# TengdaHan/CoCLR

Measured on AMD Instinct MI355X. Metric: clips/sec (whole node) S3D-InfoNCE seq_len=32 bs=32/GPU, higher is better.
Workload: dtype fp32

## Files before the change

coclr_amd/csrc/pool.hip:

```cpp
#include "common.h"
#include "../../include/coclr_hip.h"
#include <math.h>
#include <cstdlib>

namespace {

struct PoolGeom {
  int N, C;
  int Ti, Hi, Wi, To, Ho, Wo;
  int kt, kh, kw, st, sh, sw, pt, ph, pw;
  long x_nstride, y_nstride;
  const float* in_scale;
  const float* in_shift;
  int in_relu;
  int C0;
  int tfold;
  int nt;
};

typedef float pool_f32x4 __attribute__((ext_vector_type(4)));

__device__ __forceinline__ float4 pool_ld4(const float* p, int i, bool nt) {
  if (nt) {
    const pool_f32x4 t = __builtin_nontemporal_load(reinterpret_cast<const pool_f32x4*>(p) + i);
    return make_float4(t.x, t.y, t.z, t.w);
  }
  return reinterpret_cast<const float4*>(p)[i];
}
__device__ __forceinline__ void pool_st4(float* p, int i, const float4& w, bool nt) {
  if (nt) {
    pool_f32x4 t; t.x = w.x; t.y = w.y; t.z = w.z; t.w = w.w;
    __builtin_nontemporal_store(t, reinterpret_cast<pool_f32x4*>(p) + i);
  } else {
    reinterpret_cast<float4*>(p)[i] = w;
  }
}
inline long pool_nt_bytes() {
  const char* e = getenv("COCLR_BN_NT_MB");
  const long mb = e ? atol(e) : 0;
  return mb < 0 ? -1 : (mb << 20);
}

__device__ __forceinline__ float pool_in(const PoolGeom& g, float v, int c) {
  if (g.in_scale) {
    v = fmaf(v, g.in_scale[c], g.in_shift[c]);
    if (g.in_relu) v = fmaxf(v, 0.f);
  }
  return v;
}

__global__ void __launch_bounds__(256)
maxpool3d_fwd_kernel(const float* __restrict__ x, float* __restrict__ y, int* __restrict__ idx,
                     const PoolGeom g) {
  const int So = g.To * g.Ho * g.Wo, Si = g.Ti * g.Hi * g.Wi;
  const int planes = g.N * g.C;
  for (int pl = blockIdx.y; pl < planes; pl += gridDim.y) {
    const int n = pl / g.C, c = pl - n * g.C;
    const float* xp = x + (long)n * g.x_nstride + (long)c * Si;
    float* yp = y + (long)n * g.y_nstride + (long)c * So;
    int* ip = idx ? idx + (long)pl * So : nullptr;
    for (int o = blockIdx.x * 256 + threadIdx.x; o < So; o += gridDim.x * 256) {
      const int ow = o % g.Wo;
      const int q = o / g.Wo;
      const int oh = q % g.Ho, ot = q / g.Ho;
      int t0 = ot * g.st - g.pt, h0 = oh * g.sh - g.ph, w0 = ow * g.sw - g.pw;
      const int t1 = min(t0 + g.kt, g.Ti), h1 = min(h0 + g.kh, g.Hi), w1 = min(w0 + g.kw, g.Wi);
      t0 = max(t0, 0); h0 = max(h0, 0); w0 = max(w0, 0);
      float best = -INFINITY;
      int bi = (t0 * g.Hi + h0) * g.Wi + w0;
      for (int t = t0; t < t1; ++t)
        for (int h = h0; h < h1; ++h)
          for (int w = w0; w < w1; ++w) {
            const int ii = (t * g.Hi + h) * g.Wi + w;
            const float v = pool_in(g, xp[ii], c);
            if (v > best || v != v) { best = v; bi = ii; }
          }
      yp[o] = best;
      if (ip) ip[o] = bi;
    }
  }
}

__device__ __forceinline__ int first_out(int a, int s) { return a < 0 ? 0 : a / s + 1; }

__global__ void __launch_bounds__(256)
maxpool3d_bwd_kernel(const float* __restrict__ dy, const int* __restrict__ idx, float* dx,
                     const PoolGeom g, long dy_nstride, long dx_nstride, int accumulate) {
  const int So = g.To * g.Ho * g.Wo, Si = g.Ti * g.Hi * g.Wi;
  const int planes = g.N * g.C;
  for (int pl = blockIdx.y; pl < planes; pl += gridDim.y) {
    const int n = pl / g.C, c = pl - n * g.C;
    const float* dyp = dy + (long)n * dy_nstride + (long)c * So;
    const int* ip = idx + (long)pl * So;
    float* dxp = dx + (long)n * dx_nstride + (long)c * Si;
    for (int i = blockIdx.x * 256 + threadIdx.x; i < Si; i += gridDim.x * 256) {
      const int iw = i % g.Wi;
      const int q = i / g.Wi;
      const int ih = q % g.Hi, it = q / g.Hi;
      const int ot0 = first_out(it + g.pt - g.kt, g.st);
      const int oh0 = first_out(ih + g.ph - g.kh, g.sh);
      const int ow0 = first_out(iw + g.pw - g.kw, g.sw);
      const int ot1 = min(g.To - 1, (it + g.pt) / g.st);
      const int oh1 = min(g.Ho - 1, (ih + g.ph) / g.sh);
      const int ow1 = min(g.Wo - 1, (iw + g.pw) / g.sw);
      float s = 0.f;
      for (int ot = ot0; ot <= ot1; ++ot)
        for (int oh = oh0; oh <= oh1; ++oh)
          for (int ow = ow0; ow <= ow1; ++ow) {
            const int o = (ot * g.Ho + oh) * g.Wo + ow;
            if (ip[o] == i) s += dyp[o];
          }
      dxp[i] = accumulate ? dxp[i] + s : s;
    }
  }
}

template <int KT, int KH, int KW, int ST, int SH, int SW, int WPT, bool WITH_IDX>
__global__ void __launch_bounds__(256)
maxpool3d_tiled_fwd_kernel(const float* __restrict__ x, float* __restrict__ y,
                           int* __restrict__ idx, const PoolGeom g, int G, int planes, int tfold,
                           int vec) {
  extern __shared__ float tile[];
  const int Si = g.Ti * g.Hi * g.Wi, So = g.To * g.Ho * g.Wo;
  const int pl0 = blockIdx.x * G;
  const int gcount = min(G, planes - pl0);
  for (int gi = 0; gi < gcount; ++gi) {
    const int pl = pl0 + gi;
    const int n = pl / g.C, c = pl - n * g.C;
    const float* xp = x + (long)n * g.x_nstride + (long)c * Si;
    float* tp = tile + gi * Si;
    const int ch = c / g.tfold;
    if (vec) {
      for (int i = threadIdx.x; i < (Si >> 2); i += 256) {
        float4 v = pool_ld4(xp, i, g.nt != 0);
        v.x = pool_in(g, v.x, ch); v.y = pool_in(g, v.y, ch);
        v.z = pool_in(g, v.z, ch); v.w = pool_in(g, v.w, ch);
        reinterpret_cast<float4*>(tp)[i] = v;
      }
    } else {
      for (int i = threadIdx.x; i < Si; i += 256) tp[i] = pool_in(g, xp[i], ch);
    }
  }
  __syncthreads();
  constexpr int NR = (WPT - 1) * SW + KW;
  const int OWC = (g.Wo + WPT - 1) / WPT;
  const int rows = g.To * g.Ho;
  const int items = gcount * rows * OWC;
  for (int it = threadIdx.x; it < items; it += 256) {
    const int owc = it % OWC;
    int r = it / OWC;
    const int oh = r % g.Ho; r /= g.Ho;
    const int ot = r % g.To;
    const int gi = r / g.To;
    const int ow0 = owc * WPT;
    const float* tp = tile + gi * Si;
    float best[WPT];
    int bi[WPT];
    const int t0 = ot * ST - g.pt, h0 = oh * SH - g.ph, w0 = ow0 * SW - g.pw;
#pragma unroll
    for (int j = 0; j < WPT; ++j) {
      best[j] = -INFINITY;
      const int tt = max(t0, 0), hh = max(h0, 0), ww = max(w0 + j * SW, 0);
      bi[j] = (tt * g.Hi + hh) * g.Wi + ww;
    }
#pragma unroll
    for (int kt = 0; kt < KT; ++kt) {
      const int t = t0 + kt;
      if (t < 0 || t >= g.Ti) continue;
#pragma unroll
      for (int kh = 0; kh < KH; ++kh) {
        const int h = h0 + kh;
        if (h < 0 || h >= g.Hi) continue;
        const int rowoff = (t * g.Hi + h) * g.Wi;
        float v[NR];
#pragma unroll
        for (int q = 0; q < NR; ++q) {
          const int w = w0 + q;
          v[q] = (w >= 0 && w < g.Wi) ? tp[rowoff + w] : -INFINITY;
        }
#pragma unroll
        for (int j = 0; j < WPT; ++j) {
#pragma unroll
          for (int kw = 0; kw < KW; ++kw) {
            const float val = v[j * SW + kw];
            if (val > best[j] || val != val) { best[j] = val; bi[j] = rowoff + w0 + j * SW + kw; }
          }
        }
      }
    }
    const int pl = pl0 + gi;
    const int n = pl / g.C, c = pl - n * g.C;
    const long obase = ((long)ot * g.Ho + oh) * g.Wo + ow0;
    float* yp = y + (long)n * g.y_nstride + (long)c * So + obase;
#pragma unroll
    for (int j = 0; j < WPT; ++j) {
      if (ow0 + j < g.Wo) {
        yp[j] = best[j];
        if (WITH_IDX) idx[(long)pl * So + obase + j] = bi[j] + (pl % tfold) * Si;
      }
    }
  }
}

template <int PT, int PH, int PW, int KQ>
struct ClassLoads {
  int i[PT * PH * PW][KQ];
  int b[PT * PH * PW][KQ];
  float v[PT * PH * PW][KQ];
};

template <int PT, int PH, int PW, int KQ>
__device__ __forceinline__ void class_load(ClassLoads<PT, PH, PW, KQ>& L, const float* __restrict__ dy,
                                           const int* __restrict__ idx, const PoolGeom& g,
                                           long dy_nstride, int pl0, int gcount, int tfold, int Si,
                                           int So) {
#pragma unroll
  for (int ct = 0; ct < PT; ++ct)
#pragma unroll
    for (int ch = 0; ch < PH; ++ch)
#pragma unroll
      for (int cw = 0; cw < PW; ++cw) {
        const int cls = (ct * PH + ch) * PW + cw;
        const int nt = (g.To - ct + PT - 1) / PT, nh = (g.Ho - ch + PH - 1) / PH,
                  nw = (g.Wo - cw + PW - 1) / PW;
        const int csize = (nt > 0 && nh > 0 && nw > 0) ? nt * nh * nw : 0;
#pragma unroll
        for (int k = 0; k < KQ; ++k) {
          const int q = threadIdx.x + k * 256;
          L.i[cls][k] = -1;
          L.b[cls][k] = 0;
          L.v[cls][k] = 0.f;
          if (q < gcount * csize) {
            const int gi = q / csize;
            int m = q - gi * csize;
            const int a = m / (nh * nw);
            m -= a * nh * nw;
            const int b = m / nw, cc = m - b * nw;
            const int o = ((a * PT + ct) * g.Ho + (b * PH + ch)) * g.Wo + (cc * PW + cw);
            const int pl = pl0 + gi;
            const int n = pl / g.C, c = pl - n * g.C;
            L.b[cls][k] = gi * Si - (pl % tfold) * Si;
            L.i[cls][k] = idx[(long)pl * So + o];
            L.v[cls][k] = dy[(long)n * dy_nstride + (long)c * So + o];
          }
        }
      }
}

template <int PT, int PH, int PW, int KQ>
__device__ __forceinline__ void class_apply(const ClassLoads<PT, PH, PW, KQ>& L, float* tile) {
#pragma unroll
  for (int cls = 0; cls < PT * PH * PW; ++cls) {
    asm volatile("s_waitcnt lgkmcnt(0)\n\ts_barrier" ::: "memory");
#pragma unroll
    for (int k = 0; k < KQ; ++k)
      if (L.i[cls][k] >= 0) tile[L.b[cls][k] + L.i[cls][k]] += L.v[cls][k];
  }
}

__device__ __forceinline__ void class_scatter_generic(float* tile, const float* __restrict__ dy,
                                                      const int* __restrict__ idx, const PoolGeom& g,
                                                      long dy_nstride, int pl0, int gcount, int tfold,
                                                      int Si, int So) {
  const int Pt = (g.kt + g.st - 1) / g.st, Ph = (g.kh + g.sh - 1) / g.sh, Pw = (g.kw + g.sw - 1) / g.sw;
  for (int ct = 0; ct < Pt; ++ct)
    for (int ch = 0; ch < Ph; ++ch)
      for (int cw = 0; cw < Pw; ++cw) {
        __syncthreads();
        const int nt = (g.To - ct + Pt - 1) / Pt, nh = (g.Ho - ch + Ph - 1) / Ph,
                  nw = (g.Wo - cw + Pw - 1) / Pw;
        if (nt <= 0 || nh <= 0 || nw <= 0) continue;
        const int csize = nt * nh * nw;
        for (int q = threadIdx.x; q < gcount * csize; q += 256) {
          const int gi = q / csize;
          int m = q - gi * csize;
          const int a = m / (nh * nw);
          m -= a * nh * nw;
          const int b = m / nw, cc = m - b * nw;
          const int o = ((a * Pt + ct) * g.Ho + (b * Ph + ch)) * g.Wo + (cc * Pw + cw);
          const int pl = pl0 + gi;
          const int n = pl / g.C, c = pl - n * g.C;
          const int i = idx[(long)pl * So + o] - (pl % tfold) * Si;
          tile[gi * Si + i] += dy[(long)n * dy_nstride + (long)c * So + o];
        }
      }
}

template <int PT, int PH, int PW, int KQ>
__global__ void __launch_bounds__(256)
maxpool3d_tiled_bwd_kernel(const float* __restrict__ dy, const int* __restrict__ idx, float* dx,
                           const PoolGeom g, long dy_nstride, long dx_nstride, int accumulate,
                           int G, int planes, int tfold, int vec) {
  extern __shared__ float tile[];
  const int Si = g.Ti * g.Hi * g.Wi, So = g.To * g.Ho * g.Wo;
  const int pl0 = blockIdx.x * G;
  const int gcount = min(G, planes - pl0);
  if constexpr (PT > 0) {
    ClassLoads<PT, PH, PW, KQ> L;
    class_load<PT, PH, PW, KQ>(L, dy, idx, g, dy_nstride, pl0, gcount, tfold, Si, So);
    for (int i = threadIdx.x; i < gcount * Si; i += 256) tile[i] = 0.f;
    class_apply<PT, PH, PW, KQ>(L, tile);
  } else {
    for (int i = threadIdx.x; i < gcount * Si; i += 256) tile[i] = 0.f;
    class_scatter_generic(tile, dy, idx, g, dy_nstride, pl0, gcount, tfold, Si, So);
  }
  __syncthreads();
  for (int gi = 0; gi < gcount; ++gi) {
    const int pl = pl0 + gi;
    const int n = pl / g.C, c = pl - n * g.C;
    float* dxp = dx + (long)n * dx_nstride + (long)c * Si;
    const float* tp = tile + gi * Si;
    if (vec) {
      for (int i = threadIdx.x; i < (Si >> 2); i += 256) {
        float4 v = reinterpret_cast<const float4*>(tp)[i];
        if (accumulate) {
          const float4 o = reinterpret_cast<const float4*>(dxp)[i];
          v.x += o.x; v.y += o.y; v.z += o.z; v.w += o.w;
        }
        reinterpret_cast<float4*>(dxp)[i] = v;
      }
    } else {
      for (int i = threadIdx.x; i < Si; i += 256) dxp[i] = accumulate ? dxp[i] + tp[i] : tp[i];
    }
  }
}


struct PoolBest { float v; int i; };

__device__ __forceinline__ void pool_take(PoolBest& b, float cv, int ci) {
  if (cv > b.v || cv != cv) { b.v = cv; b.i = ci; }
}

template <bool WITH_IDX, int TT>
__global__ void __launch_bounds__(256)
maxpool333_kernel(const float* __restrict__ x, float* __restrict__ y, int* __restrict__ idx,
                  const PoolGeom g, int planes, int lW, int lHW, int vec) {
  extern __shared__ float lds[];
  const int T = TT > 0 ? TT : g.Ti;
  const int W = 1 << lW, HW = 1 << lHW, H = HW >> lW;
  const int PG = 256 >> lHW, S = T << lHW;
  float* xs = lds;
  float* bv = xs + PG * S;
  int* bi = reinterpret_cast<int*>(bv + PG * S);
  const int tid = threadIdx.x;
  const int pl0 = blockIdx.x * PG;
  const int gcount = min(PG, planes - pl0);
  if (vec) {
    const int S4 = S >> 2, total4 = gcount * S4;
    for (int e0 = tid; e0 < total4; e0 += 4 * 256) {
      float4 r[4];
      int chn[4];
#pragma unroll
      for (int k = 0; k < 4; ++k) {
        const int e = e0 + k * 256;
        chn[k] = -1;
        if (e < total4) {
          const int gi = e / S4, i = e - gi * S4;
          const int pl = pl0 + gi;
          const int n = pl / g.C, c = pl - n * g.C;
          r[k] = reinterpret_cast<const float4*>(x + (long)n * g.x_nstride + (long)c * S)[i];
          chn[k] = c;
        }
      }
#pragma unroll
      for (int k = 0; k < 4; ++k) {
        if (chn[k] < 0) continue;
        float4 v = r[k];
        v.x = pool_in(g, v.x, chn[k]); v.y = pool_in(g, v.y, chn[k]);
        v.z = pool_in(g, v.z, chn[k]); v.w = pool_in(g, v.w, chn[k]);
        reinterpret_cast<float4*>(xs)[e0 + k * 256] = v;
      }
    }
  } else {
    for (int gi = 0; gi < gcount; ++gi) {
      const int pl = pl0 + gi;
      const int n = pl / g.C, c = pl - n * g.C;
      const float* xp = x + (long)n * g.x_nstride + (long)c * S;
      float* tp = xs + gi * S;
      for (int i = tid; i < S; i += 256) tp[i] = pool_in(g, xp[i], c);
    }
  }
  __syncthreads();
  const int gl = tid >> lHW, p = tid & (HW - 1), h = p >> lW, w = p & (W - 1);
  const bool live = gl < gcount;
  if (live) {
#pragma unroll
    for (int t = 0; t < T; ++t) {
      const int row = (gl * T + t) * HW + h * W;
      const int frow = (t * H + h) * W;
      PoolBest b;
      b.v = -INFINITY;
      b.i = frow + (w > 0 ? w - 1 : 0);
      if (w > 0) pool_take(b, xs[row + w - 1], frow + w - 1);
      pool_take(b, xs[row + w], frow + w);
      if (w < W - 1) pool_take(b, xs[row + w + 1], frow + w + 1);
      bv[row + w] = b.v;
      if (WITH_IDX) bi[row + w] = b.i;
    }
  }
  __syncthreads();
  if (!live) return;
  auto plane_best = [&](int t) {
    const int col = (gl * T + t) * HW + w;
    const int h0 = h > 0 ? h - 1 : 0;
    PoolBest b;
    b.v = -INFINITY;
    b.i = WITH_IDX ? bi[col + h0 * W] : 0;
    if (h > 0) pool_take(b, bv[col + (h - 1) * W], WITH_IDX ? bi[col + (h - 1) * W] : 0);
    pool_take(b, bv[col + h * W], WITH_IDX ? bi[col + h * W] : 0);
    if (h < H - 1) pool_take(b, bv[col + (h + 1) * W], WITH_IDX ? bi[col + (h + 1) * W] : 0);
    return b;
  };
  const int pl = pl0 + gl;
  const int n = pl / g.C, c = pl - n * g.C;
  float* yp = y + (long)n * g.y_nstride + (long)c * S;
  int* ip = WITH_IDX ? idx + (long)pl * S : nullptr;
  PoolBest prev, cur = plane_best(0), next = cur;
  prev.v = -INFINITY; prev.i = cur.i;
#pragma unroll
  for (int t = 0; t < T; ++t) {
    if (t + 1 < T) next = plane_best(t + 1);
    PoolBest b;
    b.v = -INFINITY;
    b.i = t > 0 ? prev.i : cur.i;
    if (t > 0) pool_take(b, prev.v, prev.i);
    pool_take(b, cur.v, cur.i);
    if (t + 1 < T) pool_take(b, next.v, next.i);
    yp[t * HW + p] = b.v;
    if (WITH_IDX) ip[t * HW + p] = b.i;
    prev = cur;
    cur = next;
  }
}

__global__ void __launch_bounds__(256)
bn_pool_bwd_reduce_kernel(const float* __restrict__ pdy, const int* __restrict__ pidx,
                          const float* __restrict__ y, const float* __restrict__ scale,
                          const float* __restrict__ shift, const float* __restrict__ mean,
                          const float* __restrict__ invstd, double* sums, int C, int So, int Si,
                          long pdy_nstride, long y_nstride, int relu) {
  __shared__ double red[4];
  const int c = blockIdx.x, n = blockIdx.y;
  const float sc = scale[c], sf = shift[c], mu = mean[c], is = invstd[c];
  const float* dp = pdy + (long)n * pdy_nstride + (long)c * So;
  const int* ip = pidx + ((long)n * C + c) * So;
  const float* yp = y + (long)n * y_nstride + (long)c * Si;
  float ag = 0.f, agx = 0.f;
  for (int o0 = threadIdx.x; o0 < So; o0 += 1024) {
    int ii[4];
    float gg[4], vv[4];
#pragma unroll
    for (int k = 0; k < 4; ++k) {
      const int o = o0 + k * 256;
      ii[k] = o < So ? ip[o] : 0;
      gg[k] = o < So ? dp[o] : 0.f;
    }
#pragma unroll
    for (int k = 0; k < 4; ++k) vv[k] = yp[ii[k]];
#pragma unroll
    for (int k = 0; k < 4; ++k) {
      if (o0 + k * 256 >= So) break;
      float g = gg[k];
      const float v = vv[k];
      if (relu) g = fmaf(v, sc, sf) > 0.f ? g : 0.f;
      ag += g;
      agx += g * ((v - mu) * is);
    }
  }
  double sg = block256_sum_d((double)ag, red);
  double sgx = block256_sum_d((double)agx, red);
  if (threadIdx.x == 0) {
    sums[((long)c * gridDim.y + n) * 2] = sg;
    sums[((long)c * gridDim.y + n) * 2 + 1] = sgx;
  }
}

template <int PT, int PH, int PW, int KQ>
__global__ void __launch_bounds__(256)
bn_pool_bwd_apply_kernel(const float* __restrict__ pdy, const int* __restrict__ pidx,
                         const float* __restrict__ y, const float* __restrict__ scale,
                         const float* __restrict__ shift, const float* __restrict__ mean,
                         const float* __restrict__ invstd, const double* __restrict__ sums, int groups,
                         double count, int training, float* dgamma, float* dbeta, float* dy,
                         const PoolGeom g, long pdy_nstride, long y_nstride, long dy_nstride, int relu,
                         int G, int planes, int tfold, int vec) {
  extern __shared__ float tile[];
  __shared__ double tot[2];
  __shared__ float coef[8][4];
  const int Si = g.Ti * g.Hi * g.Wi, So = g.To * g.Ho * g.Wo;
  const int pl0 = blockIdx.x * G;
  const int gcount = min(G, planes - pl0);
  ClassLoads<(PT > 0 ? PT : 1), (PT > 0 ? PH : 1), (PT > 0 ? PW : 1), (PT > 0 ? KQ : 1)> L;
  if constexpr (PT > 0)
    class_load<PT, PH, PW, KQ>(L, pdy, pidx, g, pdy_nstride, pl0, gcount, tfold, Si, So);
  for (int i = threadIdx.x; i < gcount * Si; i += 256) tile[i] = 0.f;
  int cprev = -1;
  for (int gi = 0; gi < gcount; ++gi) {
    const int pl = pl0 + gi;
    const int c = (pl % g.C) / tfold;
    if (c == cprev && !(pl / g.C == 0 && (pl % g.C) % tfold == 0)) {
      if (threadIdx.x == 0)
        for (int j = 0; j < 3; ++j) coef[gi][j] = coef[gi - 1][j];
      continue;
    }
    cprev = c;
    __syncthreads();
    if (threadIdx.x < 64) {
      double a0 = 0.0, a1 = 0.0;
      for (int k = threadIdx.x; k < groups; k += 64) {
        a0 += sums[((long)c * groups + k) * 2];
        a1 += sums[((long)c * groups + k) * 2 + 1];
      }
      a0 = wave_sum_d(a0);
      a1 = wave_sum_d(a1);
      if (threadIdx.x == 0) { tot[0] = a0; tot[1] = a1; }
    }
    __syncthreads();
    if (threadIdx.x == 0) {
      const double sg = tot[0], sgx = tot[1];
      const float sc = scale[c];
      float A = sc, B = 0.f, D = 0.f;
      if (training) {
        const float mg = (float)(sg / count), mgx = (float)(sgx / count);
        B = -sc * invstd[c] * mgx;
        D = sc * (mean[c] * invstd[c] * mgx - mg);
      }
      coef[gi][0] = A; coef[gi][1] = B; coef[gi][2] = D;
      if (pl / g.C == 0 && (pl % g.C) % tfold == 0) {
        if (dgamma) dgamma[c] = (float)sgx;
        if (dbeta) dbeta[c] = (float)sg;
      }
    }
  }
  if constexpr (PT > 0) class_apply<PT, PH, PW, KQ>(L, tile);
  else class_scatter_generic(tile, pdy, pidx, g, pdy_nstride, pl0, gcount, tfold, Si, So);
  __syncthreads();
  for (int gi = 0; gi < gcount; ++gi) {
    const int pl = pl0 + gi;
    const int n = pl / g.C, c = pl - n * g.C;
    const int ch = c / tfold;
    const float A = coef[gi][0], B = coef[gi][1], D = coef[gi][2];
    const float sc = scale[ch], sf = shift[ch];
    const float* yp = y + (long)n * y_nstride + (long)c * Si;
    float* dyp = dy + (long)n * dy_nstride + (long)c * Si;
    const float* tp = tile + gi * Si;
    if (vec) {
      for (int i = threadIdx.x; i < (Si >> 2); i += 256) {
        float4 gq = reinterpret_cast<const float4*>(tp)[i];
        const float4 v = pool_ld4(yp, i, g.nt != 0);
        if (relu) {
          gq.x = fmaf(v.x, sc, sf) > 0.f ? gq.x : 0.f; gq.y = fmaf(v.y, sc, sf) > 0.f ? gq.y : 0.f;
          gq.z = fmaf(v.z, sc, sf) > 0.f ? gq.z : 0.f; gq.w = fmaf(v.w, sc, sf) > 0.f ? gq.w : 0.f;
        }
        float4 o;
        o.x = fmaf(A, gq.x, fmaf(B, v.x, D)); o.y = fmaf(A, gq.y, fmaf(B, v.y, D));
        o.z = fmaf(A, gq.z, fmaf(B, v.z, D)); o.w = fmaf(A, gq.w, fmaf(B, v.w, D));
        pool_st4(dyp, i, o, g.nt != 0);
      }
    } else {
      for (int i = threadIdx.x; i < Si; i += 256) {
        float gv = tp[i];
        const float v = yp[i];
        if (relu) gv = fmaf(v, sc, sf) > 0.f ? gv : 0.f;
        dyp[i] = fmaf(A, gv, fmaf(B, v, D));
      }
    }
  }
}

__global__ void __launch_bounds__(256)
maxpool333_bwd_kernel(const float* __restrict__ dy, const int* __restrict__ idx, float* dx,
                      const PoolGeom g, long dy_nstride, long dx_nstride, int accumulate, int G,
                      int planes, int lW, int lHW, int vec) {
  extern __shared__ float lds[];
  const int T = g.Ti, W = 1 << lW, HW = 1 << lHW, H = HW >> lW;
  const int S = T << lHW;
  float* dys = lds;
  int* ids = reinterpret_cast<int*>(lds + G * S);
  const int pl0 = blockIdx.x * G;
  const int gcount = min(G, planes - pl0);
  for (int gi = 0; gi < gcount; ++gi) {
    const int pl = pl0 + gi;
    const int n = pl / g.C, c = pl - n * g.C;
    const float* dyp = dy + (long)n * dy_nstride + (long)c * S;
    const int* ip = idx + (long)pl * S;
    if (vec) {
      for (int i = threadIdx.x; i < (S >> 2); i += 256) {
        reinterpret_cast<float4*>(dys + gi * S)[i] = reinterpret_cast<const float4*>(dyp)[i];
        reinterpret_cast<int4*>(ids + gi * S)[i] = reinterpret_cast<const int4*>(ip)[i];
      }
    } else {
      for (int i = threadIdx.x; i < S; i += 256) { dys[gi * S + i] = dyp[i]; ids[gi * S + i] = ip[i]; }
    }
  }
  __syncthreads();
  for (int q = threadIdx.x; q < gcount * S; q += 256) {
    const int gi = q / S, i = q - gi * S;
    const int t = i >> lHW, h = (i >> lW) & (H - 1), w = i & (W - 1);
    const float* dv = dys + gi * S;
    const int* iv = ids + gi * S;
    float s = 0.f;
#pragma unroll
    for (int dt = -1; dt <= 1; ++dt) {
      if (t + dt < 0 || t + dt >= T) continue;
#pragma unroll
      for (int dh = -1; dh <= 1; ++dh) {
        if (h + dh < 0 || h + dh >= H) continue;
#pragma unroll
        for (int dw = -1; dw <= 1; ++dw) {
          if (w + dw < 0 || w + dw >= W) continue;
          const int o = i + dt * HW + dh * W + dw;
          if (iv[o] == i) s += dv[o];
        }
      }
    }
    const int pl = pl0 + gi;
    const int n = pl / g.C, c = pl - n * g.C;
    float* d = dx + (long)n * dx_nstride + (long)c * S + i;
    *d = accumulate ? *d + s : s;
  }
}

constexpr int kTileFloats = 16384;

inline int pick_group(int planes, int Si) {
  if (Si > kTileFloats) return 0;
  int G = 4096 / Si;
  if (G < 1) G = 1;
  while (G > 1 && (planes + G - 1) / G < 2048) G >>= 1;
  return G;
}

template <int KT, int KH, int KW, int ST, int SH, int SW, int WPT>
int launch_tiled_fwd(const PoolGeom& g, const float* x, float* y, int* idx, int G, int planes,
                     int tfold, int vec, hipStream_t stream) {
  const size_t lds = (size_t)G * g.Ti * g.Hi * g.Wi * sizeof(float);
  const int blocks = (planes + G - 1) / G;
  if (idx) {
    auto k = maxpool3d_tiled_fwd_kernel<KT, KH, KW, ST, SH, SW, WPT, true>;
    static std::atomic<uint64_t> done{0};
    COCLR_RETURN_IF(ensure_dyn_lds(reinterpret_cast<const void*>(k), kTileFloats * 4, done));
    hipLaunchKernelGGL(k, dim3(blocks), dim3(256), lds, stream, x, y, idx, g, G, planes, tfold, vec);
  } else {
    auto k = maxpool3d_tiled_fwd_kernel<KT, KH, KW, ST, SH, SW, WPT, false>;
    static std::atomic<uint64_t> done{0};
    COCLR_RETURN_IF(ensure_dyn_lds(reinterpret_cast<const void*>(k), kTileFloats * 4, done));
    hipLaunchKernelGGL(k, dim3(blocks), dim3(256), lds, stream, x, y, idx, g, G, planes, tfold, vec);
  }
  COCLR_LAUNCH_CHECK();
  return 0;
}

inline PoolGeom fold_time(PoolGeom g) {
  if (g.kt == 1 && g.st == 1 && g.pt == 0 && g.Ti == g.To) {
    g.C = g.C * g.Ti;
    g.tfold = g.Ti;
    g.Ti = g.To = 1;
  }
  return g;
}

__global__ void __launch_bounds__(256)
global_avgpool_fwd_kernel(const float* __restrict__ x, float* __restrict__ y, int planes, int S) {
  const int wave = (blockIdx.x * 256 + threadIdx.x) >> 6, lane = threadIdx.x & 63;
  if (wave >= planes) return;
  const float* xp = x + (long)wave * S;
  float s = 0.f;
  for (int i = lane; i < S; i += 64) s += xp[i];
  s = wave_sum(s);
  if (lane == 0) y[wave] = s / (float)S;
}

__global__ void __launch_bounds__(256)
global_avgpool_bwd_kernel(const float* __restrict__ dy, float* __restrict__ dx, long total, int S) {
  const float inv = 1.f / (float)S;
  for (long e = (long)blockIdx.x * 256 + threadIdx.x; e < total; e += (long)gridDim.x * 256)
    dx[e] = dy[e / S] * inv;
}

inline dim3 pool_grid(int planes, int elems) {
  int gx = cdiv(elems, 256 * 2);
  if (gx < 1) gx = 1;
  if (gx > 128) gx = 128;
  int gy = planes > 65535 ? 65535 : planes;
  while ((long)gx * gy > 262144 && gx > 1) gx >>= 1;
  return dim3(gx, gy);
}

inline PoolGeom to_geom(const coclr_pool_desc* d) {
  PoolGeom g;
  g.N = d->N; g.C = d->C;
  g.Ti = d->Ti; g.Hi = d->Hi; g.Wi = d->Wi; g.To = d->To; g.Ho = d->Ho; g.Wo = d->Wo;
  g.kt = d->kt; g.kh = d->kh; g.kw = d->kw; g.st = d->st; g.sh = d->sh; g.sw = d->sw;
  g.pt = d->pt; g.ph = d->ph; g.pw = d->pw;
  g.x_nstride = d->x_nstride; g.y_nstride = d->y_nstride;
  g.in_scale = g.in_shift = nullptr; g.in_relu = 0; g.C0 = d->C; g.tfold = 1;
  {
    static const long nt_bytes = pool_nt_bytes();
    g.nt = (nt_bytes >= 0 && (long)d->N * d->C * d->Ti * d->Hi * d->Wi * 4 >= nt_bytes) ? 1 : 0;
  }
  return g;
}

}

static inline int ilog2_exact(int v) {
  int l = 0;
  while ((1 << l) < v) ++l;
  return (1 << l) == v ? l : -1;
}

namespace {

enum { kFwdGeneric = 0, kFwdSep333 = 1, kFwdTiled = 2 };
enum { kBwdGeneric = 0, kBwdGather333 = 1, kBwdClasses = 2 };

inline bool is_333_s1_p1(const PoolGeom& g) {
  return g.kt == 3 && g.kh == 3 && g.kw == 3 && g.st == 1 && g.sh == 1 && g.sw == 1 && g.pt == 1 && g.ph == 1 &&
         g.pw == 1;
}

struct PoolFwdPlan {
  int family;
  int tmpl;
  int G;
  int gx, gy;
  int tfold;
  int vec;
  int lds;
  int lW, lHW;
  int planes;
  PoolGeom g;
};

inline PoolFwdPlan plan_pool_fwd(const PoolGeom& g, bool with_idx) {
  PoolFwdPlan p;
  p.family = kFwdGeneric; p.tmpl = 0; p.G = 1; p.tfold = 1; p.vec = 0; p.lds = 0; p.lW = p.lHW = 0;
  p.planes = g.N * g.C;
  p.g = g;
  if (is_333_s1_p1(g)) {
    const int lW = ilog2_exact(g.Wi), lHW = ilog2_exact(g.Hi * g.Wi);
    if (lW >= 0 && lHW >= 4 && lHW <= 8 && g.Ti <= 32) {
      const int PG = 256 >> lHW, S = g.Ti << lHW;
      const size_t lds = (size_t)PG * S * 4 * (with_idx ? 3 : 2);
      if (lds <= 64 * 1024) {
        p.family = kFwdSep333;
        p.tmpl = (g.Ti == 16 || g.Ti == 8 || g.Ti == 4) ? g.Ti : 0;
        p.G = PG; p.gx = cdiv(p.planes, PG); p.gy = 1;
        p.vec = (g.x_nstride & 3) == 0;
        p.lds = (int)lds; p.lW = lW; p.lHW = lHW;
        return p;
      }
    }
  }
  {
    const PoolGeom f = fold_time(g);
    const int Si = f.Ti * f.Hi * f.Wi;
    const int planes = f.N * f.C;
    const int G = pick_group(planes, Si);
    if (G > 0) {
      const int k[3] = {f.kt, f.kh, f.kw}, s[3] = {f.st, f.sh, f.sw};
#define POOL_IS(a, b, c, e, ff, gg) (k[0] == a && k[1] == b && k[2] == c && s[0] == e && s[1] == ff && s[2] == gg)
      int row = -1;
      if (POOL_IS(1, 3, 3, 1, 2, 2)) row = 0;
      else if (POOL_IS(3, 3, 3, 1, 1, 1)) row = 1;
      else if (POOL_IS(3, 3, 3, 2, 2, 2)) row = 2;
      else if (POOL_IS(2, 2, 2, 2, 2, 2)) row = 3;
#undef POOL_IS
      if (row >= 0) {
        p.family = kFwdTiled; p.tmpl = row; p.G = G; p.gx = (planes + G - 1) / G; p.gy = 1;
        p.tfold = f.Ti == g.Ti ? 1 : g.Ti;
        p.vec = (Si & 3) == 0 && (f.x_nstride & 3) == 0;
        p.lds = (int)((size_t)G * Si * sizeof(float));
        p.planes = planes;
        p.g = f;
        return p;
      }
    }
  }
  const dim3 grid = pool_grid(g.N * g.C, g.To * g.Ho * g.Wo);
  p.gx = (int)grid.x; p.gy = (int)grid.y;
  return p;
}

}

extern "C" int coclr_maxpool3d_fwd(const coclr_pool_desc* d, const float* x, float* y,
                                   int32_t* indices, const float* in_scale, const float* in_shift,
                                   int in_relu, void* stream) {
  if (!d || d->N <= 0 || d->C <= 0) return COCLR_EINVAL;
  if (d->pt * 2 > d->kt || d->ph * 2 > d->kh || d->pw * 2 > d->kw) return COCLR_EINVAL;
  if ((in_scale == nullptr) != (in_shift == nullptr)) return COCLR_EINVAL;
  PoolGeom g = to_geom(d);
  g.in_scale = in_scale; g.in_shift = in_shift; g.in_relu = in_relu;
  const PoolFwdPlan p = plan_pool_fwd(g, indices != nullptr);
  hipStream_t st = (hipStream_t)stream;
  if (p.family == kFwdSep333) {
    const dim3 grid(p.gx);
    const size_t lds = (size_t)p.lds;
    const int planes = p.planes, lW = p.lW, lHW = p.lHW;
#define POOL333(TT)                                                                                  \
    if (indices) hipLaunchKernelGGL((maxpool333_kernel<true, TT>), grid, dim3(256), lds, st, x, y, \
                                    indices, g, planes, lW, lHW, p.vec);                         \
    else hipLaunchKernelGGL((maxpool333_kernel<false, TT>), grid, dim3(256), lds, st, x, y,       \
                            indices, g, planes, lW, lHW, p.vec)
    if (p.tmpl == 16) { POOL333(16); }
    else if (p.tmpl == 8) { POOL333(8); }
    else if (p.tmpl == 4) { POOL333(4); }
    else { POOL333(0); }
#undef POOL333
    COCLR_LAUNCH_CHECK();
    return 0;
  }
  if (p.family == kFwdTiled) {
    switch (p.tmpl) {
      case 0: return launch_tiled_fwd<1, 3, 3, 1, 2, 2, 2>(p.g, x, y, indices, p.G, p.planes, p.tfold, p.vec, st);
      case 1: return launch_tiled_fwd<3, 3, 3, 1, 1, 1, 4>(p.g, x, y, indices, p.G, p.planes, p.tfold, p.vec, st);
      case 2: return launch_tiled_fwd<3, 3, 3, 2, 2, 2, 2>(p.g, x, y, indices, p.G, p.planes, p.tfold, p.vec, st);
      default: return launch_tiled_fwd<2, 2, 2, 2, 2, 2, 2>(p.g, x, y, indices, p.G, p.planes, p.tfold, p.vec, st);
    }
  }
  hipLaunchKernelGGL(maxpool3d_fwd_kernel, dim3(p.gx, p.gy), dim3(256), 0, st, x, y, indices, g);
  COCLR_LAUNCH_CHECK();
  return 0;
}

struct ClassShape { int pt, ph, pw, kq; };
inline ClassShape class_shape(const PoolGeom& g, int G) {
  ClassShape c;
  c.pt = (g.kt + g.st - 1) / g.st; c.ph = (g.kh + g.sh - 1) / g.sh; c.pw = (g.kw + g.sw - 1) / g.sw;
  const long m = (long)((g.To + c.pt - 1) / c.pt) * ((g.Ho + c.ph - 1) / c.ph) * ((g.Wo + c.pw - 1) / c.pw);
  c.kq = (int)((G * m + 255) / 256);
  static const bool off = getenv("COCLR_POOL_PRELOAD") && atoi(getenv("COCLR_POOL_PRELOAD")) == 0;
  if (off) c.kq = 1 << 20;
  return c;
}

template <int PT, int PH, int PW, int KQ>
int launch_tiled_bwd(const float* dy, const int32_t* indices, float* dx, const PoolGeom& g,
                     long dy_nstride, long dx_nstride, int accumulate, int G, int planes, int tfold,
                     int Si, int vec, hipStream_t st) {
  auto kern = maxpool3d_tiled_bwd_kernel<PT, PH, PW, KQ>;
  static std::atomic<uint64_t> done{0};
  COCLR_RETURN_IF(ensure_dyn_lds(reinterpret_cast<const void*>(kern), kTileFloats * 4, done));
  hipLaunchKernelGGL(kern, dim3((planes + G - 1) / G), dim3(256), (size_t)G * Si * sizeof(float), st,
                     dy, indices, dx, g, dy_nstride, dx_nstride, accumulate, G, planes, tfold, vec);
  COCLR_LAUNCH_CHECK();
  return 0;
}

namespace {

struct ClassTemplate { int pt, ph, pw, kq; };
constexpr ClassTemplate kBwdTemplates[4] = {{1, 2, 2, 1}, {3, 3, 3, 1}, {2, 2, 2, 1}, {1, 1, 1, 2}};
constexpr ClassTemplate kPooledTemplates[2] = {{1, 2, 2, 1}, {2, 2, 2, 1}};

inline int pick_class_template(const ClassShape& cs, const ClassTemplate* rows, int n) {
  for (int i = 0; i < n; ++i)
    if (cs.pt == rows[i].pt && cs.ph == rows[i].ph && cs.pw == rows[i].pw && cs.kq <= rows[i].kq) return i;
  return -1;
}

struct PoolBwdPlan {
  int family;
  int tmpl;
  int G, kq;
  int gx, gy;
  int tfold;
  int vec;
  int lds;
  int lW, lHW;
  int planes, Si;
  PoolGeom g;
};

inline PoolBwdPlan plan_pool_bwd(const PoolGeom& g0, long dy_nstride, long dx_nstride) {
  PoolBwdPlan p;
  p.family = kBwdGeneric; p.tmpl = -1; p.G = 1; p.kq = 0; p.tfold = 1; p.vec = 0; p.lds = 0; p.lW = p.lHW = 0;
  p.planes = g0.N * g0.C; p.Si = g0.Ti * g0.Hi * g0.Wi;
  p.g = g0;
  if (is_333_s1_p1(g0)) {
    const int lW = ilog2_exact(g0.Wi), lHW = ilog2_exact(g0.Hi * g0.Wi);
    const int S = g0.Ti * g0.Hi * g0.Wi;
    if (lW >= 0 && lHW >= 0 && S <= 128) {
      const int planes = g0.N * g0.C;
      int G = 2048 / S;
      if (G < 1) G = 1;
      while (G > 1 && (planes + G - 1) / G < 2048) G >>= 1;
      p.family = kBwdGather333; p.G = G; p.gx = (planes + G - 1) / G; p.gy = 1;
      p.vec = (S & 3) == 0 && (dy_nstride & 3) == 0;
      p.lds = G * S * 8; p.lW = lW; p.lHW = lHW;
      return p;
    }
  }
  {
    const PoolGeom g = fold_time(g0);
    const int Si = g.Ti * g.Hi * g.Wi;
    const int planes = g.N * g.C;
    if (pick_group(planes, Si) > 0) {
      int G = 4096 / Si > 0 ? 4096 / Si : 1;
      while (G > 1 && (planes + G - 1) / G < 1024) G >>= 1;
      const ClassShape cs = class_shape(g, G);
      p.family = kBwdClasses; p.tmpl = pick_class_template(cs, kBwdTemplates, 4);
      p.G = G; p.kq = cs.kq; p.gx = (planes + G - 1) / G; p.gy = 1;
      p.tfold = g.Ti == g0.Ti ? 1 : g0.Ti;
      p.vec = (Si & 3) == 0 && (dx_nstride & 3) == 0;
      p.lds = (int)((size_t)G * Si * sizeof(float));
      p.planes = planes; p.Si = Si;
      p.g = g;
      return p;
    }
  }
  const dim3 grid = pool_grid(g0.N * g0.C, g0.Ti * g0.Hi * g0.Wi);
  p.gx = (int)grid.x; p.gy = (int)grid.y;
  return p;
}

struct PooledBnPlan {
  int fits;
  int tmpl;
  int G, kq, blocks, tfold, vec, lds, planes, Si;
  PoolGeom g;
};

inline PooledBnPlan plan_pooled_bn(const PoolGeom& g0, long y_nstride, long dy_nstride) {
  PooledBnPlan p;
  const PoolGeom g = fold_time(g0);
  p.g = g;
  p.tfold = g.Ti == g0.Ti ? 1 : g0.Ti;
  p.Si = g.Ti * g.Hi * g.Wi;
  p.planes = g.N * g.C;
  p.fits = p.Si <= kTileFloats;
  p.tmpl = -1; p.G = 0; p.kq = 0; p.blocks = 0; p.vec = 0; p.lds = 0;
  if (!p.fits) return p;
  int G = 4096 / p.Si > 0 ? 4096 / p.Si : 1;
  if (G > 8) G = 8;
  while (G > 1 && (p.planes + G - 1) / G < 1024) G >>= 1;
  const ClassShape cs = class_shape(g, G);
  p.tmpl = pick_class_template(cs, kPooledTemplates, 2);
  p.G = G; p.kq = cs.kq; p.blocks = (p.planes + G - 1) / G;
  p.vec = (p.Si & 3) == 0 && ((y_nstride | dy_nstride) & 3) == 0;
  p.lds = (int)((size_t)G * p.Si * sizeof(float));
  return p;
}

}

extern "C" int coclr_maxpool3d_bwd(const coclr_pool_desc* d, const float* dy, const int32_t* indices,
                                   float* dx, int64_t dy_nstride, int64_t dx_nstride,
                                   int accumulate, void* stream) {
  if (!d || d->N <= 0 || d->C <= 0) return COCLR_EINVAL;
  const PoolGeom g0 = to_geom(d);
  const PoolBwdPlan p = plan_pool_bwd(g0, (long)dy_nstride, (long)dx_nstride);
  hipStream_t st = (hipStream_t)stream;
  if (p.family == kBwdGather333) {
    hipLaunchKernelGGL(maxpool333_bwd_kernel, dim3(p.gx), dim3(256), (size_t)p.lds, st, dy, indices, dx, g0,
                       (long)dy_nstride, (long)dx_nstride, accumulate, p.G, p.planes, p.lW, p.lHW, p.vec);
    COCLR_LAUNCH_CHECK();
    return 0;
  }
  if (p.family == kBwdClasses) {
#define POOL_BWD(a, b, c, q)                                                                         \
    return launch_tiled_bwd<a, b, c, q>(dy, indices, dx, p.g, (long)dy_nstride, (long)dx_nstride,    \
                                        accumulate, p.G, p.planes, p.tfold, p.Si, p.vec, st)
    switch (p.tmpl) {
      case 0: POOL_BWD(1, 2, 2, 1);
      case 1: POOL_BWD(3, 3, 3, 1);
      case 2: POOL_BWD(2, 2, 2, 1);
      case 3: POOL_BWD(1, 1, 1, 2);
      default: POOL_BWD(0, 0, 0, 0);
    }
#undef POOL_BWD
  }
  hipLaunchKernelGGL(maxpool3d_bwd_kernel, dim3(p.gx, p.gy), dim3(256), 0, st, dy, indices, dx, g0,
                     (long)dy_nstride, (long)dx_nstride, accumulate);
  COCLR_LAUNCH_CHECK();
  return 0;
}

extern "C" int coclr_bn_act_backward_pooled_fits(const coclr_pool_desc* d, int* fits) {
  if (!d || !fits || d->N <= 0 || d->C <= 0) return COCLR_EINVAL;
  *fits = plan_pooled_bn(to_geom(d), 0, 0).fits;
  return 0;
}

extern "C" int coclr_bn_act_backward_pooled(const coclr_pool_desc* d, const float* pool_dy,
                                            const int32_t* pool_idx, const float* y,
                                            const float* scale, const float* shift,
                                            const float* mean, const float* invstd, double* sums,
                                            float* dy, float* dgamma, float* dbeta,
                                            int64_t pool_dy_nstride, int64_t y_nstride,
                                            int64_t dy_nstride, int relu, int training, void* stream) {
  if (!d || d->N <= 0 || d->C <= 0 || !pool_dy || !pool_idx || !y || !sums || !dy) return COCLR_EINVAL;
  const PoolGeom g0 = to_geom(d);
  const PooledBnPlan p = plan_pooled_bn(g0, (long)y_nstride, (long)dy_nstride);
  if (!p.fits) return COCLR_EINVAL;
  const PoolGeom& g = p.g;
  const int tfold = p.tfold, Si = p.Si, planes = p.planes, G = p.G;
  hipStream_t st = (hipStream_t)stream;
  const int So0 = g0.To * g0.Ho * g0.Wo, Si0 = g0.Ti * g0.Hi * g0.Wi;
  hipLaunchKernelGGL(bn_pool_bwd_reduce_kernel, dim3(g0.C, g0.N), dim3(256), 0, st, pool_dy, pool_idx,
                     y, scale, shift, mean, invstd, sums, g0.C, So0, Si0, (long)pool_dy_nstride,
                     (long)y_nstride, relu);
  COCLR_LAUNCH_CHECK();
  const double count = (double)g0.N * Si0;
#define BN_POOL_BWD(a, b, c, q)                                                                      \
  do {                                                                                               \
    auto kern = bn_pool_bwd_apply_kernel<a, b, c, q>;                                                \
    static std::atomic<uint64_t> done{0};                                                            \
    COCLR_RETURN_IF(ensure_dyn_lds(reinterpret_cast<const void*>(kern), kTileFloats * 4, done));      \
    hipLaunchKernelGGL(kern, dim3(p.blocks), dim3(256), (size_t)G * Si * sizeof(float),              \
                       st, pool_dy, pool_idx, y, scale, shift, mean, invstd, sums, g0.N, count,      \
                       training, dgamma, dbeta, dy, g, (long)pool_dy_nstride, (long)y_nstride,       \
                       (long)dy_nstride, relu, G, planes, tfold, p.vec);                             \
    COCLR_LAUNCH_CHECK();                                                                            \
    return 0;                                                                                        \
  } while (0)
  if (p.tmpl == 0) BN_POOL_BWD(1, 2, 2, 1);
  if (p.tmpl == 1) BN_POOL_BWD(2, 2, 2, 1);
  BN_POOL_BWD(0, 0, 0, 0);
#undef BN_POOL_BWD
}

extern "C" int coclr_pool_plan(const coclr_pool_desc* d, int with_indices, int64_t dy_nstride,
                               int64_t dx_nstride, int32_t out[32]) {
  if (!d || !out || d->N <= 0 || d->C <= 0) return COCLR_EINVAL;
  if (d->pt * 2 > d->kt || d->ph * 2 > d->kh || d->pw * 2 > d->kw) return COCLR_EINVAL;
  const PoolGeom g = to_geom(d);
  if (!dy_nstride) dy_nstride = (int64_t)d->C * d->To * d->Ho * d->Wo;
  if (!dx_nstride) dx_nstride = (int64_t)d->C * d->Ti * d->Hi * d->Wi;
  for (int i = 0; i < 32; ++i) out[i] = 0;
  const PoolFwdPlan f = plan_pool_fwd(g, with_indices != 0);
  out[0] = f.family; out[1] = f.tmpl; out[2] = f.G; out[3] = f.gx; out[4] = f.gy; out[5] = f.tfold;
  out[6] = f.vec; out[7] = f.lds;
  const PoolBwdPlan b = plan_pool_bwd(g, (long)dy_nstride, (long)dx_nstride);
  const ClassTemplate none = {0, 0, 0, 0};
  const ClassTemplate bt = b.tmpl >= 0 ? kBwdTemplates[b.tmpl] : none;
  out[8] = b.family; out[9] = bt.pt; out[10] = bt.ph; out[11] = bt.pw; out[12] = bt.kq; out[13] = b.G;
  out[14] = b.kq; out[15] = b.gx; out[16] = b.gy; out[17] = b.tfold; out[18] = b.vec; out[19] = b.lds;
  const PooledBnPlan q = plan_pooled_bn(g, (long)d->x_nstride, (long)dx_nstride);
  const ClassTemplate qt = q.tmpl >= 0 ? kPooledTemplates[q.tmpl] : none;
  out[20] = q.fits; out[21] = q.G; out[22] = qt.pt; out[23] = qt.ph; out[24] = qt.pw; out[25] = qt.kq;
  out[26] = q.kq; out[27] = q.blocks; out[28] = q.tfold; out[29] = q.vec; out[30] = q.lds;
  out[31] = g.nt;
  return 0;
}

extern "C" int coclr_global_avgpool_fwd(const float* x, float* y, int64_t planes, int64_t S,
                                        void* stream) {
  if (planes <= 0 || S <= 0) return COCLR_EINVAL;
  hipLaunchKernelGGL(global_avgpool_fwd_kernel, dim3(cdiv(planes * 64, 256)), dim3(256), 0,
                     (hipStream_t)stream, x, y, (int)planes, (int)S);
  COCLR_LAUNCH_CHECK();
  return 0;
}

extern "C" int coclr_global_avgpool_bwd(const float* dy, float* dx, int64_t planes, int64_t S,
                                        void* stream) {
  if (planes <= 0 || S <= 0) return COCLR_EINVAL;
  const long total = planes * S;
  int blocks = cdiv(total, 256);
  if (blocks > 2048) blocks = 2048;
  hipLaunchKernelGGL(global_avgpool_bwd_kernel, dim3(blocks), dim3(256), 0, (hipStream_t)stream, dy,
                     dx, total, (int)S);
  COCLR_LAUNCH_CHECK();
  return 0;
}
```

Before: 1150.

## Flatten small-plane pool tile loops and replace integer divides with reciprocal quotients

Replaces integer division/modulo in the tiled maxpool forward/backward kernels with float-reciprocal quotient helpers that are corrected afterwards. For small planes (under 256 float4s), tile fill and writeback loops are flattened across all planes in a block and unrolled 4x, so more threads stay busy and loads are batched. The maxpool inner window loop becomes branchless with clamped addresses and select masks. The class_load scatter is restructured so each thread loads one whole class cell group and shares a single base offset. This adds code complexity and relies on the float quotient correction staying exact.

```diff
diff --git a/coclr_amd/csrc/pool.hip b/coclr_amd/csrc/pool.hip
--- a/coclr_amd/csrc/pool.hip
+++ b/coclr_amd/csrc/pool.hip
@@ -47,6 +47,40 @@
     if (g.in_relu) v = fmaxf(v, 0.f);
   }
   return v;
+}
+
+struct PoolDiv { int d; float r; };
+__device__ __forceinline__ PoolDiv pool_div(int d) {
+  PoolDiv p;
+  p.d = d;
+  p.r = 1.f / (float)d;
+  return p;
+}
+__device__ __forceinline__ int pool_quot_small(int n, const PoolDiv& p) {
+  int q = (int)((float)n * p.r);
+  const int rem = n - q * p.d;
+  q += (rem >= p.d ? 1 : 0) - (rem < 0 ? 1 : 0);
+  return q;
+}
+__device__ __forceinline__ int pool_quot(int n, const PoolDiv& p) {
+  if (n >= (1 << 20)) return n / p.d;
+  return pool_quot_small(n, p);
+}
+
+constexpr int kSlotRunBelow = 256;
+struct PoolSlots { int S4, C, pl0; PoolDiv dS4, dC; };
+__device__ __forceinline__ PoolSlots pool_slots(int S4, int C, int pl0) {
+  PoolSlots s;
+  s.S4 = S4; s.C = C; s.pl0 = pl0;
+  s.dS4 = pool_div(S4); s.dC = pool_div(C);
+  return s;
+}
+__device__ __forceinline__ void pool_slot(const PoolSlots& s, int e, int& i, int& n, int& c) {
+  const int gi = pool_quot_small(e, s.dS4);
+  i = e - gi * s.S4;
+  const int pl = s.pl0 + gi;
+  n = pool_quot(pl, s.dC);
+  c = pl - n * s.C;
 }
 
 __global__ void __launch_bounds__(256)
@@ -124,21 +158,60 @@
   const int Si = g.Ti * g.Hi * g.Wi, So = g.To * g.Ho * g.Wo;
   const int pl0 = blockIdx.x * G;
   const int gcount = min(G, planes - pl0);
-  for (int gi = 0; gi < gcount; ++gi) {
-    const int pl = pl0 + gi;
-    const int n = pl / g.C, c = pl - n * g.C;
-    const float* xp = x + (long)n * g.x_nstride + (long)c * Si;
-    float* tp = tile + gi * Si;
-    const int ch = c / g.tfold;
-    if (vec) {
-      for (int i = threadIdx.x; i < (Si >> 2); i += 256) {
-        float4 v = pool_ld4(xp, i, g.nt != 0);
-        v.x = pool_in(g, v.x, ch); v.y = pool_in(g, v.y, ch);
-        v.z = pool_in(g, v.z, ch); v.w = pool_in(g, v.w, ch);
-        reinterpret_cast<float4*>(tp)[i] = v;
-      }
-    } else {
-      for (int i = threadIdx.x; i < Si; i += 256) tp[i] = pool_in(g, xp[i], ch);
+  const PoolDiv dC = pool_div(g.C), dfold = pool_div(tfold);
+  const int S4 = Si >> 2;
+  if (vec && S4 < kSlotRunBelow) {
+    const int total4 = gcount * S4;
+    const PoolSlots slots = pool_slots(S4, g.C, pl0);
+    for (int e0 = threadIdx.x; e0 < total4; e0 += 4 * 256) {
+      float4 r[4];
+      float sc[4], sf[4];
+      bool live[4];
+#pragma unroll
+      for (int k = 0; k < 4; ++k) {
+        const int e = e0 + k * 256;
+        live[k] = e < total4;
+        sc[k] = sf[k] = 0.f;
+        if (live[k]) {
+          int i, n, c;
+          pool_slot(slots, e, i, n, c);
+          r[k] = pool_ld4(x + (long)n * g.x_nstride + (long)c * Si, i, g.nt != 0);
+          if (g.in_scale) {
+            const int ch = pool_quot(c, dfold);
+            sc[k] = g.in_scale[ch];
+            sf[k] = g.in_shift[ch];
+          }
+        }
+      }
+#pragma unroll
+      for (int k = 0; k < 4; ++k) {
+        if (!live[k]) continue;
+        float4 v = r[k];
+        if (g.in_scale) {
+          v.x = fmaf(v.x, sc[k], sf[k]); v.y = fmaf(v.y, sc[k], sf[k]);
+          v.z = fmaf(v.z, sc[k], sf[k]); v.w = fmaf(v.w, sc[k], sf[k]);
+          if (g.in_relu) { v.x = fmaxf(v.x, 0.f); v.y = fmaxf(v.y, 0.f); v.z = fmaxf(v.z, 0.f); v.w = fmaxf(v.w, 0.f); }
+        }
+        reinterpret_cast<float4*>(tile)[e0 + k * 256] = v;
+      }
+    }
+  } else {
+    for (int gi = 0; gi < gcount; ++gi) {
+      const int pl = pl0 + gi;
+      const int n = pool_quot(pl, dC), c = pl - n * g.C;
+      const float* xp = x + (long)n * g.x_nstride + (long)c * Si;
+      float* tp = tile + gi * Si;
+      const int ch = pool_quot(c, dfold);
+      if (vec) {
+        for (int i = threadIdx.x; i < S4; i += 256) {
+          float4 v = pool_ld4(xp, i, g.nt != 0);
+          v.x = pool_in(g, v.x, ch); v.y = pool_in(g, v.y, ch);
+          v.z = pool_in(g, v.z, ch); v.w = pool_in(g, v.w, ch);
+          reinterpret_cast<float4*>(tp)[i] = v;
+        }
+      } else {
+        for (int i = threadIdx.x; i < Si; i += 256) tp[i] = pool_in(g, xp[i], ch);
+      }
     }
   }
   __syncthreads();
@@ -146,12 +219,11 @@
   const int OWC = (g.Wo + WPT - 1) / WPT;
   const int rows = g.To * g.Ho;
   const int items = gcount * rows * OWC;
+  const PoolDiv dOWC = pool_div(OWC), dHo = pool_div(g.Ho), dTo = pool_div(g.To);
   for (int it = threadIdx.x; it < items; it += 256) {
-    const int owc = it % OWC;
-    int r = it / OWC;
-    const int oh = r % g.Ho; r /= g.Ho;
-    const int ot = r % g.To;
-    const int gi = r / g.To;
+    const int r0 = pool_quot_small(it, dOWC), owc = it - r0 * OWC;
+    const int r1 = pool_quot_small(r0, dHo), oh = r0 - r1 * g.Ho;
+    const int gi = pool_quot_small(r1, dTo), ot = r1 - gi * g.To;
     const int ow0 = owc * WPT;
     const float* tp = tile + gi * Si;
     float best[WPT];
@@ -163,20 +235,32 @@
       const int tt = max(t0, 0), hh = max(h0, 0), ww = max(w0 + j * SW, 0);
       bi[j] = (tt * g.Hi + hh) * g.Wi + ww;
     }
-#pragma unroll
+    float ninf = -INFINITY;
+    asm volatile("" : "+v"(ninf));
+    int wc[NR];
+    bool wok[NR];
+#pragma unroll
+    for (int q = 0; q < NR; ++q) {
+      const int w = w0 + q;
+      wok[q] = w >= 0 && w < g.Wi;
+      wc[q] = min(max(w, 0), g.Wi - 1);
+    }
+#pragma unroll(KT * KH * NR <= 16 ? KT : 1)
     for (int kt = 0; kt < KT; ++kt) {
       const int t = t0 + kt;
-      if (t < 0 || t >= g.Ti) continue;
+      const bool tok = t >= 0 && t < g.Ti;
+      const int tcl = min(max(t, 0), g.Ti - 1);
 #pragma unroll
       for (int kh = 0; kh < KH; ++kh) {
         const int h = h0 + kh;
-        if (h < 0 || h >= g.Hi) continue;
+        const bool rok = tok && h >= 0 && h < g.Hi;
         const int rowoff = (t * g.Hi + h) * g.Wi;
+        const float* rp = tp + (tcl * g.Hi + min(max(h, 0), g.Hi - 1)) * g.Wi;
         float v[NR];
 #pragma unroll
         for (int q = 0; q < NR; ++q) {
-          const int w = w0 + q;
-          v[q] = (w >= 0 && w < g.Wi) ? tp[rowoff + w] : -INFINITY;
+          const float e = rp[wc[q]];
+          v[q] = (rok && wok[q]) ? e : ninf;
         }
 #pragma unroll
         for (int j = 0; j < WPT; ++j) {
@@ -189,14 +273,15 @@
       }
     }
     const int pl = pl0 + gi;
-    const int n = pl / g.C, c = pl - n * g.C;
+    const int n = pool_quot(pl, dC), c = pl - n * g.C;
     const long obase = ((long)ot * g.Ho + oh) * g.Wo + ow0;
     float* yp = y + (long)n * g.y_nstride + (long)c * So + obase;
+    const int fold_off = WITH_IDX ? (pl - pool_quot(pl, dfold) * tfold) * Si : 0;
 #pragma unroll
     for (int j = 0; j < WPT; ++j) {
       if (ow0 + j < g.Wo) {
         yp[j] = best[j];
-        if (WITH_IDX) idx[(long)pl * So + obase + j] = bi[j] + (pl % tfold) * Si;
+        if (WITH_IDX) idx[(long)pl * So + obase + j] = bi[j] + fold_off;
       }
     }
   }
@@ -205,8 +290,8 @@
 template <int PT, int PH, int PW, int KQ>
 struct ClassLoads {
   int i[PT * PH * PW][KQ];
-  int b[PT * PH * PW][KQ];
   float v[PT * PH * PW][KQ];
+  int b[KQ];
 };
 
 template <int PT, int PH, int PW, int KQ>
@@ -214,37 +299,43 @@
                                            const int* __restrict__ idx, const PoolGeom& g,
                                            long dy_nstride, int pl0, int gcount, int tfold, int Si,
                                            int So) {
-#pragma unroll
-  for (int ct = 0; ct < PT; ++ct)
-#pragma unroll
-    for (int ch = 0; ch < PH; ++ch)
-#pragma unroll
-      for (int cw = 0; cw < PW; ++cw) {
-        const int cls = (ct * PH + ch) * PW + cw;
-        const int nt = (g.To - ct + PT - 1) / PT, nh = (g.Ho - ch + PH - 1) / PH,
-                  nw = (g.Wo - cw + PW - 1) / PW;
-        const int csize = (nt > 0 && nh > 0 && nw > 0) ? nt * nh * nw : 0;
-#pragma unroll
-        for (int k = 0; k < KQ; ++k) {
-          const int q = threadIdx.x + k * 256;
+  const int mt = (g.To + PT - 1) / PT, mh = (g.Ho + PH - 1) / PH, mw = (g.Wo + PW - 1) / PW;
+  const int msize = mt * mh * mw;
+  const PoolDiv dsize = pool_div(msize), dhw = pool_div(mh * mw), dw = pool_div(mw);
+  const PoolDiv dC = pool_div(g.C), dfold = pool_div(tfold);
+#pragma unroll
+  for (int k = 0; k < KQ; ++k) {
+    const int q = threadIdx.x + k * 256;
+    const bool live = q < gcount * msize;
+    const int gi = live ? pool_quot_small(q, dsize) : 0;
+    int m = live ? q - gi * msize : 0;
+    const int a = pool_quot_small(m, dhw);
+    m -= a * mh * mw;
+    const int b = pool_quot_small(m, dw), cc = m - b * mw;
+    const int t0 = a * PT, h0 = b * PH, w0 = cc * PW;
+    const int o0 = (t0 * g.Ho + h0) * g.Wo + w0;
+    const int pl = pl0 + gi;
+    const int n = pool_quot(pl, dC), c = pl - n * g.C;
+    const int* ip = idx + (long)pl * So + o0;
+    const float* dp = dy + (long)n * dy_nstride + (long)c * So + o0;
+    L.b[k] = gi * Si - (pl - pool_quot(pl, dfold) * tfold) * Si;
+#pragma unroll
+    for (int ct = 0; ct < PT; ++ct)
+#pragma unroll
+      for (int ch = 0; ch < PH; ++ch)
+#pragma unroll
+        for (int cw = 0; cw < PW; ++cw) {
+          const int cls = (ct * PH + ch) * PW + cw;
+          const int off = (ct * g.Ho + ch) * g.Wo + cw;
+          const bool has = live && t0 + ct < g.To && h0 + ch < g.Ho && w0 + cw < g.Wo;
           L.i[cls][k] = -1;
-          L.b[cls][k] = 0;
           L.v[cls][k] = 0.f;
-          if (q < gcount * csize) {
-            const int gi = q / csize;
-            int m = q - gi * csize;
-            const int a = m / (nh * nw);
-            m -= a * nh * nw;
-            const int b = m / nw, cc = m - b * nw;
-            const int o = ((a * PT + ct) * g.Ho + (b * PH + ch)) * g.Wo + (cc * PW + cw);
-            const int pl = pl0 + gi;
-            const int n = pl / g.C, c = pl - n * g.C;
-            L.b[cls][k] = gi * Si - (pl % tfold) * Si;
-            L.i[cls][k] = idx[(long)pl * So + o];
-            L.v[cls][k] = dy[(long)n * dy_nstride + (long)c * So + o];
+          if (has) {
+            L.i[cls][k] = ip[off];
+            L.v[cls][k] = dp[off];
           }
         }
-      }
+  }
 }
 
 template <int PT, int PH, int PW, int KQ>
@@ -254,7 +345,7 @@
     asm volatile("s_waitcnt lgkmcnt(0)\n\ts_barrier" ::: "memory");
 #pragma unroll
     for (int k = 0; k < KQ; ++k)
-      if (L.i[cls][k] >= 0) tile[L.b[cls][k] + L.i[cls][k]] += L.v[cls][k];
+      if (L.i[cls][k] >= 0) tile[L.b[k] + L.i[cls][k]] += L.v[cls][k];
   }
 }
 
@@ -305,13 +396,42 @@
     class_scatter_generic(tile, dy, idx, g, dy_nstride, pl0, gcount, tfold, Si, So);
   }
   __syncthreads();
+  const PoolDiv dC = pool_div(g.C);
+  const int S4 = Si >> 2;
+  if (vec && S4 < kSlotRunBelow) {
+    const int total4 = gcount * S4;
+    const PoolSlots slots = pool_slots(S4, g.C, pl0);
+    for (int e0 = threadIdx.x; e0 < total4; e0 += 4 * 256) {
+      float4 o[4];
+      float* dp[4];
+#pragma unroll
+      for (int k = 0; k < 4; ++k) {
+        const int e = e0 + k * 256;
+        dp[k] = nullptr;
+        if (e < total4) {
+          int i, n, c;
+          pool_slot(slots, e, i, n, c);
+          dp[k] = dx + (long)n * dx_nstride + (long)c * Si + 4 * i;
+          if (accumulate) o[k] = *reinterpret_cast<const float4*>(dp[k]);
+        }
+      }
+#pragma unroll
+      for (int k = 0; k < 4; ++k) {
+        if (!dp[k]) continue;
+        float4 v = reinterpret_cast<const float4*>(tile)[e0 + k * 256];
+        if (accumulate) { v.x += o[k].x; v.y += o[k].y; v.z += o[k].z; v.w += o[k].w; }
+        *reinterpret_cast<float4*>(dp[k]) = v;
+      }
+    }
+    return;
+  }
   for (int gi = 0; gi < gcount; ++gi) {
     const int pl = pl0 + gi;
-    const int n = pl / g.C, c = pl - n * g.C;
+    const int n = pool_quot(pl, dC), c = pl - n * g.C;
     float* dxp = dx + (long)n * dx_nstride + (long)c * Si;
     const float* tp = tile + gi * Si;
     if (vec) {
-      for (int i = threadIdx.x; i < (Si >> 2); i += 256) {
+      for (int i = threadIdx.x; i < S4; i += 256) {
         float4 v = reinterpret_cast<const float4*>(tp)[i];
         if (accumulate) {
           const float4 o = reinterpret_cast<const float4*>(dxp)[i];
@@ -536,10 +656,11 @@
   if constexpr (PT > 0) class_apply<PT, PH, PW, KQ>(L, tile);
   else class_scatter_generic(tile, pdy, pidx, g, pdy_nstride, pl0, gcount, tfold, Si, So);
   __syncthreads();
+  const PoolDiv dC = pool_div(g.C), dfold = pool_div(tfold);
   for (int gi = 0; gi < gcount; ++gi) {
     const int pl = pl0 + gi;
-    const int n = pl / g.C, c = pl - n * g.C;
-    const int ch = c / tfold;
+    const int n = pool_quot(pl, dC), c = pl - n * g.C;
+    const int ch = pool_quot(c, dfold);
     const float A = coef[gi][0], B = coef[gi][1], D = coef[gi][2];
     const float sc = scale[ch], sf = shift[ch];
     const float* yp = y + (long)n * y_nstride + (long)c * Si;
```

New measurement: 1165 (median of 6 runs). +1.3%, better.
